# microsoft/Tokenizer

Measured on AMD Instinct MI355X. Metric: input MB/s encoded (cl100k_base), higher is better.
Workload: dtype u8

## Files before the change

tokenizer_amd/csrc/tkz_api.cpp:

```cpp
#include <algorithm>
#include <cstdio>
#include <cstdlib>
#include <cstring>
#include <atomic>
#include <chrono>
#include <memory>
#include <mutex>
#include <thread>
#include <string>
#include <unordered_map>
#include <unordered_set>
#include <vector>

#include "../../include/tkz.h"
#include "tkz_adapt.h"
#include "tkz_bpe.h"
#include "tkz_corpus.h"
#include "tkz_kernels.h"
#include "tkz_pretok.h"
#include "tkz_promo_select.h"
#include "tkz_sdma.h"
#include "tkz_vocab.h"

namespace {
// ... 650 lines not shown
constexpr int64_t kForkMaxLong = int64_t(1) << 20;
constexpr int64_t kForkMaxLongTail = int64_t(1) << 21, kForkTailShare = 2048;
void side_streams(tkz_encoder* e, Workspace* ws, int64_t total, tkz::Launch* L) {
    const bool short_queue = ws->last_lq_total >= 0 && (ws->last_lq_total <= kForkMaxLong || (ws->last_lq_total <= kForkMaxLongTail && ws->last_coop * kForkTailShare >= ws->last_lq_total));
    if (total <= e->latency_bytes || !short_queue) return;
    if (!ws->fork_token) { int none = 0; ws->fork_token = g_fork_in_flight.compare_exchange_strong(none, 1); }
    bool ok = ws->fork_token;
    for (hipStream_t* st : {&ws->st_side, &ws->st_side2}) if (!*st && hipStreamCreateWithFlags(st, hipStreamNonBlocking) != hipSuccess) { *st = nullptr; ok = false; }
    for (hipEvent_t* ev : {&ws->ev_fork, &ws->ev_join, &ws->ev_join2}) if (!*ev && hipEventCreateWithFlags(ev, hipEventDisableTiming) != hipSuccess) { *ev = nullptr; ok = false; }
    if (ok) { L->side = ws->st_side; L->side2 = ws->st_side2; L->ev_fork = ws->ev_fork; L->ev_join = ws->ev_join; L->ev_join2 = ws->ev_join2; }
    else (void)hipGetLastError();
}

int64_t sizing_sample(int64_t ntiles) {
    int64_t min_sub = (int64_t(64) << 20) / tkz::kSub;
    { const char* v = getenv("TKZ_SIZING_MIN_SUB"); if (v && atoll(v) > 0) min_sub = atoll(v); }
    return ntiles >= min_sub ? std::min<int64_t>(ntiles, std::max<int64_t>(ntiles / 16, min_sub / 16)) : -1;
}

tkz_status arm_learning(tkz_encoder* e, Workspace* ws, const BatchCall& c, bool first, TkzTables* T) {
    using namespace tkz;
    const int64_t total = c.total;
    const hipStream_t stream = c.stream;
    {
        std::lock_guard<std::mutex> lock(e->mu);
        bool others = false;
        for (Workspace* w : e->pool) if (w != ws && w->busy) others = true;
        const AdaptPolicy::Arm arm = e->policy.may_learn(total, first && !ws->learning, c.may_learn(), e->T.memo_n != 0, e->T.max_rank < (int32_t)kPromoFlag, e->promo_items.size(), others);
        if (arm != AdaptPolicy::Arm::No && e->t_memo_hits.ensure((size_t)e->memo_slots * 4, &e->bytes_allocated) == hipSuccess &&
            e->t_long_log.ensure((size_t)kLongLogCap * kLongLogDwords * 4 + 64, &e->bytes_allocated) == hipSuccess) {
            const bool clear = arm == AdaptPolicy::Arm::YesClearMemo;
            if (!clear || (hipMemsetAsync(e->t_memo.p, 0, size_t(e->memo_slots) * sizeof(TkzMemoSlot), stream) == hipSuccess && hipStreamSynchronize(stream) == hipSuccess)) {
                ws->learn_window_start = e->policy.window_armed(clear);
                ws->learning = true;
            }
        }
        *T = e->T;
    }
    if (ws->learning) {
        T->memo_hits = e->t_memo_hits.as<uint32_t>();
        T->memo_hits_sparse = total >= (int64_t(64) << 20) ? 1u : 0u;
        if (ws->learn_window_start && first) {
            HIP_TRY(hipMemsetAsync(T->memo_hits, 0, (size_t)e->memo_slots * 4, stream));
            HIP_TRY(hipMemsetAsync(e->t_long_log.as<char>() + (size_t)kLongLogCap * kLongLogDwords * 4, 0, 64, stream));
        }
    }
    return TKZ_OK;
}

tkz::EncodeParams bind_params(Workspace* ws, const uint8_t* d_bytes, const int64_t* d_offs, int64_t n_docs, int64_t total) {
    using namespace tkz;
    char* cb = ws->w_counters.as<char>();
    EncodeParams P{};
    P.bytes = d_bytes; P.total = total; P.startbits = ws->w_startbits.as<uint64_t>(); P.docbits = ws->w_docbits.as<uint64_t>(); P.nwords = total / 64 + 1;
    P.offs = d_offs; P.n_docs = n_docs;
    P.tmp = ws->w_tmp.as<int32_t>(); P.dense = ws->w_dense.as<int32_t>(); P.tile_count = ws->w_tcount.as<int32_t>();
    P.prank = ws->w_prank.as<int32_t>(); P.prank_cap = (int64_t)(ws->w_prank.cap / 4); P.pcount = ws->w_pcount.as<int32_t>(); P.pbase = ws->w_pbase.as<int64_t>();
    P.mlist = ws->w_mlist.as<uint32_t>(); P.mquad = ws->w_mquad.as<uint4>(); P.mcap = ws->mcap; P.mcount = ws->w_mcount.as<uint32_t>();
    P.docord_base = ws->w_dbase.as<int64_t>(); P.doc_tok = ws->w_doctok.as<int32_t>(); P.counters = ws->w_counters.as<int32_t>();
    P.giant_q = ws->w_gq.as<int64_t>(); P.giant_cap = total / kArenaPiece + 1; P.giant_cnt = ws->w_gcnt.as<int32_t>();
    P.giant_count = reinterpret_cast<unsigned long long*>(cb + offsetof(CounterBlock, heavy_count));
    P.giant_ticket = reinterpret_cast<unsigned long long*>(cb + offsetof(CounterBlock, giant_ticket));
    P.heavy_flag = ws->w_heavyq.as<uint8_t>(); P.nsub = (total + kSub - 1) / kSub;
    P.pool = ws->w_pool.as<int32_t>(); P.pool_head = reinterpret_cast<unsigned long long*>(cb + offsetof(CounterBlock, pool_head)); P.pool_cap = (int64_t)(ws->w_pool.cap / 4);
    return P;
}

#ifdef TKZ_DEVPROF
unsigned long long* g_devprof = nullptr;
tkz_status devprof_arm(tkz::EncodeParams* P, hipStream_t stream) {
    { const char* ab = getenv("TKZ_DEV_ABLATE"); P->ablate = ab ? atoi(ab) : 0; }
    if (P->ablate & 16) {
        if (!g_devprof) { HIP_TRY(hipMalloc((void**)&g_devprof, 64 * 8)); }
        HIP_TRY(hipMemsetAsync(g_devprof, 0, 64 * 8, stream));
    }
    P->devprof = g_devprof;
    return TKZ_OK;
}
tkz_status devprof_report() {
    if (!g_devprof || !getenv("TKZ_DEV_ABLATE") || !(atoi(getenv("TKZ_DEV_ABLATE")) & 16)) return TKZ_OK;
    unsigned long long h[64];
    HIP_TRY(hipMemcpy(h, g_devprof, sizeof h, hipMemcpyDeviceToHost));
    const double w = h[0] ? (double)h[0] : 1.0;
    fprintf(stderr, "[tkz devprof] k_probe waves %llu  clock ticks/wave: total %.0f  load+compact %.0f  short batches %.0f  mid batches %.0f | mid pieces/wave %.1f pieces/wave %.1f\n",
            h[0], h[1] / w, h[2] / w, h[3] / w, h[4] / w, h[5] / w, h[6] / w);
    if (h[51]) fprintf(stderr, "[tkz devprof] k_probe lane-cycle table, per sub-tile: load+compact %.0f ticks (64 lanes) | 13+-byte pre-pass %.0f ticks, %.1f pieces in %.2f passes of 64 (lane use %.3f) | main loop: first bucket %.0f ticks at lane use %.3f (%.2f batches of 64, %.1f pieces), second bucket %.0f ticks for %.1f lanes (%.3f of the lanes of the iterations that run it: %.2f of %.2f iterations), records and lists %.0f ticks at lane use %.3f\n",
                       h[2] / w, h[4] / w, h[5] / w, (double)((h[5] + 63 * h[0]) / 64) / w, h[5] ? (double)h[5] / (64.0 * (double)((h[5] + 63 * h[0]) / 64)) : 0.0,
                       h[48] / w, (double)h[52] / (64.0 * (double)h[51]), h[51] / w, h[52] / w, h[49] / w, h[53] / w, h[54] ? (double)h[53] / (128.0 * (double)h[54]) : 0.0, h[54] / w, (double)((h[51] + 1) / 2) / w,
                       h[50] / w, (double)h[52] / (64.0 * (double)h[51]));
    if (h[8]) fprintf(stderr, "[tkz devprof] k_giant_merge pieces %llu  clock ticks/piece: rounds in global memory %.0f  the tail %.0f | bytes/piece %.0f tokens/piece %.0f | slowest piece %llu ticks | global rounds/piece %.2f | parts/piece when the tail took over %.0f\n",
                      h[8], (double)h[9] / h[8], (double)h[10] / h[8], (double)h[11] / h[8], (double)h[12] / h[8], h[13], (double)h[14] / h[8], (double)h[7] / h[8]);
    if (h[8]) fprintf(stderr, "[tkz devprof] slowest giant piece: %llu bytes -> %llu tokens, global rounds %llu (%llu ticks), bytes first/middle/last %02llx %02llx %02llx\n",
                      h[24], h[27], h[25], h[28], h[29] & 255, (h[29] >> 8) & 255, (h[29] >> 16) & 255);
    if (h[32]) fprintf(stderr, "[tkz devprof] k_merge_long waves %llu units %llu  ticks/wave %.0f | of all ticks: sort %.3f batch formation %.3f bytes %.3f first level %.3f merges %.3f emission %.3f | fast batches %llu lanes/batch %.1f steps/batch %.1f merges/lane %.2f lane use in the merge loop %.3f ticks/step %.0f\n",
                       h[32], h[44], (double)h[33] / h[32], (double)h[34] / h[33], (double)h[35] / h[33], (double)h[36] / h[33], (double)h[37] / h[33], (double)h[38] / h[33], (double)h[39] / h[33],
                       h[40], (double)h[41] / (h[40] ? h[40] : 1), (double)h[42] / (h[40] ? h[40] : 1), (double)h[43] / (h[41] ? h[41] : 1), (double)h[43] / (64.0 * (h[42] ? h[42] : 1)), (double)h[38] / (h[42] ? h[42] : 1));
    if (h[16]) fprintf(stderr, "[tkz devprof] tail: batches %llu merges %llu (%.2f a batch) proposals/batch %.1f | rounds for chains of equal pairs %llu | ticks/batch %.0f | longest tail: %llu batches, %llu ticks\n",
                       h[16], h[17], (double)h[17] / h[16], (double)h[18] / h[16], h[19], (double)h[22] / h[16], h[20], h[23]);
    return TKZ_OK;
}
#else
tkz_status devprof_arm(tkz::EncodeParams*, hipStream_t) { return TKZ_OK; }
tkz_status devprof_report() { return TKZ_OK; }
#endif

tkz_status enqueue_attempt(tkz_encoder* e, Workspace* ws, const tkz::Launch& L, const TkzTables& T, const BatchCall& c, bool marks_reused, int64_t nsample,
                           bool* pieces_over) {
    using namespace tkz;
    const hipStream_t stream = L.stream;
    const uint8_t* const d_bytes = c.d_bytes;
    const int64_t* const d_offs = c.d_offs;
    const int64_t n_docs = c.n_docs, total = c.total;
    PiecesOut* const po = c.pieces;
    const int64_t nwords = total / 64 + 1, ntiles = (total + kSub - 1) / kSub;
    int32_t* counters = ws->w_counters.as<int32_t>();
    char* cb = ws->w_counters.as<char>();
    uint64_t* docbits = ws->w_docbits.as<uint64_t>();
    uint64_t* startbits = ws->w_startbits.as<uint64_t>();
    const SpecialCall* const special = c.literals();
    if (marks_reused) {
        HIP_TRY(hipMemsetAsync(ws->w_zero.p, 0, 256, stream));
        if (!c.bitmap_only()) HIP_TRY(hipMemsetAsync(ws->w_heavyq.p, 0, (size_t)(ws->w_zero.as<char>() + ws->zero_bytes - ws->w_heavyq.as<char>()), stream));
    } else {
        if (c.ingest) launch_ingest(L, c.ingest->h_bytes, total, const_cast<uint8_t*>(d_bytes), c.ingest->h_offs, n_docs + 1, const_cast<int64_t*>(d_offs), ws->w_zero.p, (int64_t)ws->zero_bytes);
        else if (ws->zero_bytes <= (size_t(8) << 20)) launch_ingest(L, nullptr, 0, nullptr, nullptr, 0, nullptr, ws->w_zero.p, (int64_t)ws->zero_bytes);
        else HIP_TRY(hipMemsetAsync(ws->w_zero.p, 0, ws->zero_bytes, stream));
        launch_docmark(L, d_offs, n_docs, total, docbits, counters);
        const uint64_t* isobits = docbits;
        const int64_t* iso_offs = d_offs;
        int64_t n_iso = n_docs;
        if (special) {
            for (DevBuf* b : {&ws->w_candbits, &ws->w_segbits, &ws->w_specbits, &ws->w_endbits}) HIP_TRY(b->ensure((size_t)(nwords + 8) * 8, &ws->bytes_allocated));
            launch_lit_scan(L, d_bytes, total, docbits, nwords, e->LIT, special->allowed, ws->w_candbits.as<uint64_t>(), ws->w_segbits.as<uint64_t>(),
                            ws->w_specbits.as<uint64_t>(), ws->w_endbits.as<uint64_t>(), reinterpret_cast<unsigned long long*>(cb + offsetof(CounterBlock, n_literals)), c.d_repl);
            isobits = ws->w_segbits.as<uint64_t>();
            if (e->pretok_seq || e->pattern == TKZ_PATTERN_O200K || e->pattern == TKZ_PATTERN_O200K_DOTNET) {
                int64_t* nseg = reinterpret_cast<int64_t*>(cb + offsetof(CounterBlock, ndocstarts));
                launch_doccount2(L, isobits, isobits, nwords, total, ntiles, ws->w_dcount.as<int32_t>(), ws->w_pcount.as<int32_t>());
                launch_scan2(L, ntiles, ws->w_bsum.as<int64_t>(), ws->w_dcount.as<int32_t>(), ws->w_dbase.as<int64_t>(), nseg, 1, nullptr, nullptr, nullptr, 1, -1);
                HIP_TRY(hipMemcpyAsync(&ws->h_counters->ndocstarts, nseg, 8, hipMemcpyDeviceToHost, stream));
                HIP_TRY(hipStreamSynchronize(stream));
                ws->n_seg = ws->h_counters->ndocstarts;
                HIP_TRY(ws->w_segoffs.ensure((size_t)(ws->n_seg + 2) * 8, &ws->bytes_allocated));
                launch_seg_offsets(L, isobits, nwords, total, ntiles, ws->w_dbase.as<int64_t>(), ws->n_seg, ws->w_segoffs.as<int64_t>());
                iso_offs = ws->w_segoffs.as<int64_t>();
                n_iso = ws->n_seg;
            }
        }
        if (!c.pretokenizes()) {
            HIP_TRY(hipMemcpyAsync(startbits, docbits, (size_t)nwords * 8, hipMemcpyDeviceToDevice, stream));
        } else if (e->pretok_seq) {
            HIP_TRY(hipMemcpyAsync(startbits, isobits, (size_t)nwords * 8, hipMemcpyDeviceToDevice, stream));
            launch_pretok_seq(L, e->pattern, d_bytes, iso_offs, n_iso, total, startbits, T.bmp_class, counters);
        } else {
            HIP_TRY(ws->w_xq.ensure((size_t)(nwords / kRowsPerWave + 4) * 16, &ws->bytes_allocated));
            launch_pretok_rows(L, e->pattern, d_bytes, iso_offs, n_iso, total, isobits, startbits, nwords, T.bmp_class, counters,
                               ws->w_xq.as<int64_t>(), reinterpret_cast<unsigned long long*>(cb + offsetof(CounterBlock, xcount)));
        }
        if (c.pretokenizes() && e->case_equiv && e->pattern == TKZ_PATTERN_CL100K) launch_case_equiv_fix(L, d_bytes, total, isobits, startbits);
        if (special) launch_lit_fix(L, startbits, isobits, ws->w_specbits.as<uint64_t>(), ws->w_endbits.as<uint64_t>(), nwords);
    }
    if (c.bitmap_only()) {
        HIP_TRY(hipMemcpyAsync(c.d_bitmap, startbits, (size_t)nwords * 8, hipMemcpyDeviceToDevice, stream));
    } else {
        EncodeParams P = bind_params(ws, d_bytes, d_offs, n_docs, total);
        P.lane_piece = kLanePiece;
        P.latency = total <= e->latency_bytes ? 1 : 0;
        P.tc_atomic = (L.side || P.latency) ? 1 : 0;
        if (L.side && nsample < 0) ++ws->forked_batches;
        P.coop_cap = total / P.lane_piece + 64;
// ... 1945 lines not shown
```

tokenizer_amd/csrc/tkz_kernels.hip:

```cpp
#include "tkz_kernels.h"

#include <type_traits>

#include "tkz_bpe.h"
#include "tkz_classes.h"
#include "tkz_corpus.h"
#include "tkz_pretok.h"
#include "tkz_simt.h"

namespace tkz {

TKZ_KERNEL(256) void k_docmark(const int64_t* offs, int64_t n_items, int64_t total, uint64_t* bits, int32_t* counters) {
    const int64_t stride = simt::nblocks() * simt::nthreads();
    for (int64_t d = simt::bid() * simt::nthreads() + simt::tid(); d <= n_items; d += stride) {
        const int64_t pos = offs[d];
        bool ok = pos >= 0 && pos <= total;
        if (d == 0) ok = ok && pos == 0;
        if (d == n_items) ok = ok && pos == total;
        else ok = ok && pos <= offs[d + 1];
        if (!ok) { simt::atomic_or((unsigned*)&counters[0], (unsigned)kErrOffsets); continue; }
        const int64_t w = pos >> 6;
        if (d > 0) { const int64_t prev = offs[d - 1]; if (prev >= 0 && prev <= pos && (prev >> 6) == w) continue; }
        uint64_t m = 1ull << (pos & 63);
        int64_t cur = pos;
// ... 352 lines not shown
        if (lane == 0) st = start0;
        int bad = 0;
        if (t0 < b1) {
            int64_t v = t0;
            int64_t d = doc_of(v);
            if (lane == 0) { for (int back = 0; v > offs[d] && v > wlo && back < 3 && (wb(v) & 0xC0) == 0x80; ++back) --v; }
            else { for (int k = 0; k < 3 && v < t1 && v > offs[d] && v < offs[d + 1] && (wb(v) & 0xC0) == 0x80; ++k) ++v; }
            while (v < t1) {
                while (offs[d + 1] <= v) ++d;
                const int64_t a = offs[d], e = offs[d + 1];
                TkzDoc doc; doc.b = win + (a - wlo); doc.n = (e < cut ? e : cut) - a; doc.bmp = bmp; doc.by_code_point = pattern == TKZ_PAT_O200K;
                const TkzChar ch = tkz_doc_char(doc, v - a);
                bad |= ch.bad;
                v += ch.len;
            }
        }
        if (simt::ballot(bad != 0)) { if (lane == 0) simt::atomic_or((unsigned*)&counters[0], (unsigned)kErrUtf8); continue; }
        if (st < lim) {
            int64_t pos = st, d = doc_of(st), curw = -1;
            uint64_t acc = 0;
            while (pos < lim) {
                while (offs[d + 1] <= pos) ++d;
                const int64_t a = offs[d], e = offs[d + 1];
                TkzDoc doc; doc.b = win + (a - wlo); doc.n = (e < cut ? e : cut) - a; doc.bmp = bmp; doc.by_code_point = pattern == TKZ_PAT_O200K;
                if (pos >= b0) {
                    if ((pos >> 6) != curw) {
                        if (acc) simt::atomic_or64((unsigned long long*)&startbits[curw], acc);
                        curw = pos >> 6; acc = 0;
                    }
                    acc |= 1ull << (pos & 63);
                }
                pos = a + tkz_match_at(pattern, doc, pos - a);
            }
            if (acc) simt::atomic_or64((unsigned long long*)&startbits[curw], acc);
        }
    }
}

TKZ_KERNEL(256) void k_pretok_seq(const uint8_t* bytes, const int64_t* offs, int64_t n_docs, int64_t total, uint64_t* startbits,
                                  int pattern, const uint8_t* bmp, int32_t* counters) {
    const int64_t stride = simt::nblocks() * simt::nthreads();
    for (int64_t d = simt::bid() * simt::nthreads() + simt::tid(); d < n_docs; d += stride) {
        const int64_t a = offs[d], b = offs[d + 1];
        if (b <= a || a < 0 || b > total) continue;
        TkzDoc doc; doc.b = bytes + a; doc.n = b - a; doc.bmp = bmp; doc.by_code_point = pattern == TKZ_PAT_O200K;
        int bad = 0;
        for (int64_t p = 0; p < doc.n;) { const TkzChar c = tkz_doc_char(doc, p); bad |= c.bad; p += c.len; }
        if (bad) { simt::atomic_or((unsigned*)&counters[0], (unsigned)kErrUtf8); continue; }
        int64_t curw = -1; uint64_t acc = 0;
        for (int64_t p = 0; p < doc.n;) {
            const int64_t g = a + p;
            if ((g >> 6) != curw) {
                if (acc) simt::atomic_or64((unsigned long long*)&startbits[curw], acc);
                curw = g >> 6; acc = 0;
            }
            acc |= 1ull << (g & 63);
            p = tkz_match_at(pattern, doc, p);
        }
        if (acc) simt::atomic_or64((unsigned long long*)&startbits[curw], acc);
    }
}

constexpr uint32_t kPrMiss = 1u << 31, kPrMark = 1u << 30, kPrLong = 1u << 29, kPrGiant = 1u << 28;
constexpr uint32_t kPrRankMask = (1u << 28) - 1u;
constexpr uint32_t kMrDone = 1u << 31, kMrDense = 1u << 30, kMrInline = 1u << 29;
constexpr int kMrLenShift = 10, kMrCntShift = 12;
constexpr uint32_t kMrOffMask = (1u << kMrCntShift) - 1u;
static_assert(kDenseCap <= (1 << kMrCntShift) && kSub <= (1 << kMrLenShift), "the offset field of a result entry");
#ifndef TKZ_PROBE_U
#define TKZ_PROBE_U 2
#endif
#ifndef TKZ_MS_THREADS
#define TKZ_MS_THREADS 256
#endif
#ifndef TKZ_PROBE_OCC
#define TKZ_PROBE_OCC 8
#endif
constexpr int kGroup = kMergeGroup;
constexpr int kMsThreads = TKZ_MS_THREADS;
#ifndef TKZ_PROBE_PER
#define TKZ_PROBE_PER 1
#endif
constexpr int kProbePer = TKZ_PROBE_PER;
constexpr int kMidMax = kSub / (TKZ_SHORT_KEY_MAX + 1) + 2;

TKZ_DEV int64_t tkz_xcd_block(int64_t b, int64_t nblocks) { return (b & 7) * (nblocks >> 3) + (b >> 3); }

template <int BITS>
TKZ_DEV int tkz_wave_scan(int v, int* total) {
    const uint64_t below = tkz_lowmask(simt::lane());
    int pre = 0, tot = 0;
#pragma unroll
    for (int j = 0; j < BITS; ++j) {
        const uint64_t m = simt::ballot((v >> j) & 1);
        pre += tkz_popc64(m & below) << j;
        tot += tkz_popc64(m) << j;
    }
    *total = tot;
    return pre;
}

TKZ_DEV int tkz_wave_scan_sum(int v, int* total) {
    const int x = simt::scan_inclusive(v);
    *total = simt::last_lane(x);
    return x - v;
}

TKZ_DEV uint32_t tkz_key_dword(const uint32_t* s_bytes, int s, int len, int i) {
    const int w = (s >> 2) + i;
    const uint32_t x = simt::alignbit(s_bytes[w + 1], s_bytes[w], (uint32_t)(s & 3) * 8u);
    const int nb = len - 4 * i;
    return nb >= 4 ? x : (nb <= 0 ? 0u : (x & ((1u << (8 * nb)) - 1u)));
}

constexpr int kProbeLdsBytes = (kSub + kHalo) + 2 * (kSub + 2) + 2 * kMidMax + 4 * kMidMax + 4 * (kSub / 32);
constexpr int kProbeLdsQuads = (kProbeLdsBytes + 15) / 16;
struct ProbeLds { uint32_t* bytes; uint16_t* pstart; uint16_t* mid; uint32_t* midres; uint32_t* mark; const uint4* kmask; uint32_t* spec ; };
TKZ_DEV ProbeLds tkz_probe_lds(uint4* wave_quads, const uint4* kmask) {
    ProbeLds L;
    uint8_t* b = reinterpret_cast<uint8_t*>(wave_quads);
    L.bytes = reinterpret_cast<uint32_t*>(b); b += kSub + kHalo;
    L.midres = reinterpret_cast<uint32_t*>(b); b += 4 * kMidMax;
    L.mark = reinterpret_cast<uint32_t*>(b); b += 4 * (kSub / 32);
    L.pstart = reinterpret_cast<uint16_t*>(b); b += 2 * (kSub + 2);
    L.mid = reinterpret_cast<uint16_t*>(b);
    L.kmask = kmask;
    L.spec = nullptr;
    return L;
}
TKZ_DEV void tkz_probe_kmask_init(uint4* s_kmask) {
    if (simt::tid() <= TKZ_SHORT_KEY_MAX) {
        const int len = simt::tid();
        uint32_t m[3];
        for (int i = 0; i < 3; ++i) { const int nb = len - 4 * i; m[i] = nb >= 4 ? 0xFFFFFFFFu : (nb <= 0 ? 0u : ((1u << (8 * nb)) - 1u)); }
        uint4 v; v.x = m[0]; v.y = m[1]; v.z = m[2]; v.w = 0;
        s_kmask[len] = v;
    }
}
struct ProbeText { uint4 v0, v1; };
static_assert((kSub + kHalo) / 16 <= 128, "two 16-byte loads per lane cover the sub-tile and its halo");
TKZ_DEV void tkz_probe_request_text(const EncodeParams& P, int64_t sub, ProbeText* tx) {
    const int lane = simt::lane();
    const int64_t base = sub * kSub;
    uint4 v0, v1;
    v0.x = v0.y = v0.z = v0.w = 0; v1 = v0;
    const int64_t p0 = base + 16 * (int64_t)lane, p1 = base + 16 * (int64_t)(lane + 64);
    if (p0 + 16 <= P.total) v0 = tkz_load16_nt(P.bytes + p0);
    else {
        uint32_t w[4] = {0, 0, 0, 0};
        for (int j = 0; j < 16; ++j) if (p0 + j < P.total) w[j >> 2] |= (uint32_t)P.bytes[p0 + j] << (8 * (j & 3));
        v0.x = w[0]; v0.y = w[1]; v0.z = w[2]; v0.w = w[3];
    }
    if (lane + 64 < (kSub + kHalo) / 16) {
        if (p1 + 16 <= P.total) v1 = tkz_load16_nt(P.bytes + p1);
        else {
            uint32_t w[4] = {0, 0, 0, 0};
            for (int j = 0; j < 16; ++j) if (p1 + j < P.total) w[j >> 2] |= (uint32_t)P.bytes[p1 + j] << (8 * (j & 3));
            v1.x = w[0]; v1.y = w[1]; v1.z = w[2]; v1.w = w[3];
        }
    }
    tx->v0 = v0; tx->v1 = v1;
}
TKZ_DEV bool tkz_bits_any(const uint64_t* rw, int64_t nrw, int64_t bit, int len) {
    const int64_t wa = bit >> 6, wb = (bit + len - 1) >> 6;
    for (int64_t w = wa; w <= wb && w < nrw; ++w) {
        uint64_t m = rw[w];
        if (w == wa) m &= ~tkz_lowmask((int)(bit & 63));
        if (w == wb) m &= tkz_lowmask((int)((bit + len - 1) & 63) + 1);
        if (m) return true;
    }
    return false;
}
TKZ_DEV bool tkz_lit_replaced(const uint32_t* meta, int i, const uint64_t* rw, int64_t nrw, int64_t bit, int len) {
    return rw && ((meta[kLitFffdHead + (i >> 5)] >> (i & 31)) & 1u) && tkz_bits_any(rw, nrw, bit, len);
}
TKZ_DEV int32_t tkz_lit_id(const EncodeParams& P, const uint8_t* sb, const uint8_t* gb, int s, int len, int64_t abs) {
    const uint8_t* tx = s + len <= kSub + kHalo ? sb + s : gb + s;
    for (int i = 0; i < P.n_lit; ++i) {
        const uint32_t m = P.lit_meta[kLitMetaHead + 2 * i];
        if ((int)(m >> 16) != len) continue;
        const uint8_t* lit = P.lit_blob + (m & 0xFFFFu);
        int k = 0;
        while (k < len && lit[k] == tx[k]) ++k;
        if (k == len && !tkz_lit_replaced(P.lit_meta, i, P.lit_repl, P.nwords, abs, len)) return (int32_t)P.lit_meta[kLitMetaHead + 2 * i + 1];
    }
    return TKZ_RANK_NONE;
}
template <bool REPORT, bool SPECIAL = false>
TKZ_DEV void tkz_probe_subtile(const TkzTables& T, const EncodeParams& P, int64_t sub, const ProbeLds& LD, ProbeText& tx, int64_t next) {
    const int lane = simt::lane();
    uint32_t* s_bytes = LD.bytes;
    uint16_t* s_pstart = LD.pstart;
    uint16_t* s_mid = LD.mid;
    uint32_t* s_midres = LD.midres;
    uint32_t* s_mark = LD.mark;
    const uint4* s_kmask = LD.kmask;
    const uint8_t* sb = reinterpret_cast<const uint8_t*>(s_bytes);
    const int64_t base = sub * kSub;
    const int nb = (int)(P.total - base < kSub ? P.total - base : kSub);
    const uint8_t* gbase = P.bytes + base;
    const bool prof = TKZ_DEV_FLAG(P, 16);
    long long t_0 = prof ? simt::clock() : 0, t_1 = 0, t_2 = 0, t_3 = 0;
    uint4 v0 = tx.v0, v1 = tx.v1;
    uint64_t myword = 0, mymark = 0;
    uint64_t myspec = 0;
    if (lane < kSub / 64) {
        const int64_t w = sub * (kSub / 64) + lane;
        if (w < P.nwords) { myword = P.startbits[w]; mymark = P.docbits[w]; if (SPECIAL) myspec = P.specbits[w]; }
    }
    const int64_t from = base + nb, w0 = from >> 6;
    uint64_t ahead = (w0 + lane < P.nwords) ? P.startbits[w0 + lane] : 0ull;
    const int64_t pb = P.pbase[sub];
    { uint4* s4 = reinterpret_cast<uint4*>(s_bytes); s4[lane] = v0; if (lane + 64 < (kSub + kHalo) / 16) s4[lane + 64] = v1; }
    if (next >= 0) tkz_probe_request_text(P, next, &tx);
    if (lane < kSub / 64) {
        const int lim = nb - lane * 64;
        if (lim <= 0) myword = 0; else if (lim < 64) myword &= tkz_lowmask(lim);
        s_mark[2 * lane] = (uint32_t)mymark; s_mark[2 * lane + 1] = (uint32_t)(mymark >> 32);
        if (SPECIAL) { LD.spec[2 * lane] = (uint32_t)myspec; LD.spec[2 * lane + 1] = (uint32_t)(myspec >> 32); }
    }
    int64_t last_end;
    {
        int64_t found = -1;
        for (int64_t c = 0; found < 0; ++c) {
            const int64_t w = w0 + c * 64 + lane;
            uint64_t v = c == 0 ? ahead : (w < P.nwords ? P.startbits[w] : 0);
            if (w == w0) v &= ~tkz_lowmask((int)(from & 63));
            const uint64_t any = simt::ballot(v != 0);
            if (any) {
                const int src = tkz_ctz64(any);
                const uint32_t lo = simt::shflu((uint32_t)v, src), hi = simt::shflu((uint32_t)(v >> 32), src);
                found = ((w0 + c * 64 + src) << 6) + tkz_ctz64(((uint64_t)hi << 32) | lo);
            } else if (w0 + (c + 1) * 64 >= P.nwords) found = P.total;
        }
        last_end = found;
    }
    const int last_end_rel = (int)(last_end - base < 2 * kSub + 2 ? last_end - base : 2 * kSub + 2);
    const uint32_t wlo = simt::shflu((uint32_t)myword, lane >> 2), whi = simt::shflu((uint32_t)(myword >> 32), lane >> 2);
    const uint32_t bits16 = (uint32_t)(((((uint64_t)whi << 32) | wlo) >> (16 * (lane & 3))) & 0xFFFFull);
    int np;
    {
        int off = tkz_wave_scan<5>(tkz_popc32(bits16), &np);
        for (uint32_t b = bits16; b; b &= b - 1) s_pstart[off++] = (uint16_t)(16 * lane + tkz_ctz32(b));
        if (lane == 0) s_pstart[np] = (uint16_t)last_end_rel;
    }
    (void)simt::ballot(true);
    if (prof) t_1 = simt::clock();
    const char* tb0 = reinterpret_cast<const char*>(T.short_slots);
    const uint32_t mid_off = (uint32_t)(reinterpret_cast<const char*>(T.mid_slots) - tb0);
    int nmid = 0;
#pragma unroll 1
    for (int k0 = 0; k0 < np; k0 += 64) {
        const int k = k0 + lane;
        int len = 0;
        if (k < np) len = (int)s_pstart[k + 1] - (int)s_pstart[k];
        const uint64_t midm = simt::ballot(len > TKZ_SHORT_KEY_MAX && len <= kArenaPiece);
        if ((midm >> lane) & 1ull) s_mid[nmid + tkz_popc64(midm & tkz_lowmask(lane))] = (uint16_t)k;
        nmid += tkz_popc64(midm);
    }
    (void)simt::ballot(true);
#pragma unroll 1
    for (int m0 = 0; m0 < nmid; m0 += 64) {
        const bool valid = m0 + lane < nmid;
        int s = 0, len = 13;
        uint32_t kk[7] = {0, 0, 0, 0, 0, 0, 0}, oa = 0, ob = 0;
        if (valid) {
            const int k = s_mid[m0 + lane];
            s = s_pstart[k];
            len = (int)s_pstart[k + 1] - s;
        }
        const bool is_lit = SPECIAL && valid && ((LD.spec[s >> 5] >> (s & 31)) & 1u);
        const bool is_mid = valid && len <= TKZ_MID_KEY_MAX && !is_lit;
        if (is_mid) {
#pragma unroll
            for (int i = 0; i < 7; ++i) kk[i] = tkz_key_dword(s_bytes, s, len, i);
            uint32_t s1, s2;
            tkz_mid_slots(T, kk, (uint32_t)len, &s1, &s2);
            oa = mid_off + 32u * s1; ob = mid_off + 32u * s2;
        }
        const uint4 a0 = tkz_load16(tb0 + oa), a1 = tkz_load16(tb0 + oa + 16u), b0 = tkz_load16(tb0 + ob), b1 = tkz_load16(tb0 + ob + 16u);
        int32_t rank = TKZ_RANK_NONE;
        if (is_mid) rank = tkz_match_mid(kk, (uint32_t)len, a0, a1, b0, b1);
        else if (is_lit) rank = tkz_lit_id(P, sb, gbase, s, len, base + s);
        else if (valid) {
            if (s + len <= kSub + kHalo) rank = tkz_lookup_long(T, [&](int i) -> uint32_t { return sb[s + i]; }, (uint32_t)len);
            else rank = tkz_lookup_long(T, [&](int i) -> uint32_t { return gbase[s + i]; }, (uint32_t)len);
        }
        if (valid) s_midres[m0 + lane] = (uint32_t)rank;
    }
    (void)simt::ballot(true);
    if (prof) t_2 = simt::clock();
    uint32_t* const ml = P.mlist + sub * (int64_t)P.mcap;
    uint4* const mq = P.mquad + sub * (int64_t)P.mcap;
    int ns = 0, nl = 0, midseen = 0;
    int promo_extra = 0;
    bool giant = false, coopl = false;
    constexpr int U = TKZ_PROBE_U;
#ifdef TKZ_DEVPROF
    long long pf_first = 0, pf_second = 0, pf_emit = 0, pf_t = 0;
    int pf_batches = 0, pf_valid = 0, pf_want2 = 0, pf_iters2 = 0;
#define TKZ_PROBE_MARK(acc) do { if (prof) { const long long pf_now = simt::clock(); acc += pf_now - pf_t; pf_t = pf_now; } } while (0)
    if (prof) pf_t = simt::clock();
#else
#define TKZ_PROBE_MARK(acc) do { } while (0)
#endif
#pragma unroll 1
    for (int k0 = 0; k0 < np; k0 += 64 * U) {
        int ps[U], plen[U];
        uint32_t hs[U], kw0[U], kw1[U], kw2[U];
        uint4 a0[U], a1[U];
#pragma unroll
        for (int u = 0; u < U; ++u) {
            const int k = k0 + 64 * u + lane;
            ps[u] = 0; plen[u] = 0;
            if (k < np) { ps[u] = s_pstart[k]; plen[u] = (int)s_pstart[k + 1] - ps[u]; }
            const int s = ps[u], w = s >> 2;
            const uint32_t sh = (uint32_t)(s & 3) * 8u;
            const uint32_t d0 = s_bytes[w], d1 = s_bytes[w + 1], d2 = s_bytes[w + 2], d3 = s_bytes[w + 3];
            const bool is_short = plen[u] >= 1 && plen[u] <= TKZ_SHORT_KEY_MAX;
            const uint4 km = s_kmask[is_short ? plen[u] : 0];
            kw0[u] = simt::alignbit(d1, d0, sh) & km.x; kw1[u] = simt::alignbit(d2, d1, sh) & km.y; kw2[u] = simt::alignbit(d3, d2, sh) & km.z;
            const uint32_t slot = tkz_short_slot_first(T, kw0[u], kw1[u], kw2[u], (uint32_t)plen[u], &hs[u]);
            const uint32_t oa = is_short ? 16u * slot : 0u;
            a0[u] = tkz_load16(tb0 + oa); a1[u] = tkz_load16(tb0 + oa + 16u);
        }
        int32_t rk[U];
        bool more = false;
#pragma unroll
        for (int u = 0; u < U; ++u) {
            const bool is_short = plen[u] >= 1 && plen[u] <= TKZ_SHORT_KEY_MAX;
            rk[u] = tkz_match_short2x(kw0[u], kw1[u], kw2[u], (uint32_t)plen[u], a0[u], a1[u]);
            if (SPECIAL && is_short && ((LD.spec[ps[u] >> 5] >> (ps[u] & 31)) & 1u)) rk[u] = tkz_lit_id(P, sb, gbase, ps[u], plen[u], base + ps[u]);
            more = more || (is_short && rk[u] == TKZ_RANK_NONE);
        }
        bool two_pass = simt::ballot(more) != 0;
        TKZ_PROBE_MARK(pf_first);
#ifdef TKZ_DEVPROF
        if (prof) {
            for (int u = 0; u < U; ++u) { const int nv = np - (k0 + 64 * u); if (nv > 0) { ++pf_batches; pf_valid += nv < 64 ? nv : 64; } }
            for (int u = 0; u < U; ++u) pf_want2 += tkz_popc64(simt::ballot(plen[u] >= 1 && plen[u] <= TKZ_SHORT_KEY_MAX && rk[u] == TKZ_RANK_NONE));
            pf_iters2 += two_pass ? 1 : 0;
            pf_t = simt::clock();
        }
#endif
        if (two_pass) {
#pragma unroll
            for (int u = 0; u < U; ++u) {
                const bool want = plen[u] >= 1 && plen[u] <= TKZ_SHORT_KEY_MAX && rk[u] == TKZ_RANK_NONE;
                if (want) {
                    const uint32_t ob = 16u * tkz_short_slot_second(T, hs[u]);
                    a0[u] = tkz_load16(tb0 + ob); a1[u] = tkz_load16(tb0 + ob + 16u);
                }
            }
#pragma unroll
            for (int u = 0; u < U; ++u) {
                const bool want = plen[u] >= 1 && plen[u] <= TKZ_SHORT_KEY_MAX && rk[u] == TKZ_RANK_NONE;
                if (want) rk[u] = tkz_match_short2x(kw0[u], kw1[u], kw2[u], (uint32_t)plen[u], a0[u], a1[u]);
            }
        }
        TKZ_PROBE_MARK(pf_second);
#pragma unroll
        for (int u = 0; u < U; ++u) {
            const int k = k0 + 64 * u + lane;
            const bool valid = k < np;
            const int s = ps[u], len = plen[u];
            const bool is_mid = len > TKZ_SHORT_KEY_MAX && len <= kArenaPiece;
            const uint64_t midm = simt::ballot(is_mid);
            int32_t rank = rk[u];
            if (is_mid) rank = (int32_t)s_midres[midseen + tkz_popc64(midm & tkz_lowmask(lane))];
            midseen += tkz_popc64(midm);
            const bool is_giant = len > kArenaPiece;
            const bool miss = valid && !is_giant && rank == TKZ_RANK_NONE;
            if (P.pextra) {
                const uint32_t ex = (valid && !is_giant && !miss && ((uint32_t)rank & kPromoFlag)) ? (((uint32_t)rank >> kPromoCntShift) & 3u) : 0u;
                promo_extra += (int)ex;
            }
            const bool miss_s = miss && len <= kShortMax, miss_l = miss && len > kShortMax;
            const uint64_t sm = simt::ballot(miss_s), lm = simt::ballot(miss_l);
            const int is_ = ns + tkz_popc64(sm & tkz_lowmask(lane)), il = nl + tkz_popc64(lm & tkz_lowmask(lane));
            ns += tkz_popc64(sm); nl += tkz_popc64(lm);
            const uint32_t ent = (uint32_t)s | ((uint32_t)(len - 1) << kMrLenShift);
            if (miss_s && is_ + nl < P.mcap) {
                ml[is_] = ent;
                uint4 kq; kq.x = kw0[u]; kq.y = kw1[u]; kq.z = kw2[u]; kq.w = 0;
                if (len > TKZ_SHORT_KEY_MAX) { kq.x = tkz_key_dword(s_bytes, s, len, 0); kq.y = tkz_key_dword(s_bytes, s, len, 1); kq.z = tkz_key_dword(s_bytes, s, len, 2); kq.w = tkz_key_dword(s_bytes, s, len, 3); }
                mq[is_] = kq;
            }
            if (miss_l && il + ns < P.mcap) ml[P.mcap - 1 - il] = ent;
            uint32_t rec = ((s_mark[s >> 5] >> (s & 31)) & 1u) ? kPrMark : 0u;
            if (REPORT) giant = giant || (miss_l && len > kSmallLanePiece);
            else coopl = coopl || (miss_l && len > P.lane_piece);
            if (is_giant) { rec |= kPrMiss | kPrGiant | (uint32_t)s; giant = giant || valid; }
            else if (miss) rec |= kPrMiss | (miss_l ? (kPrLong | (uint32_t)il) : (uint32_t)is_);
            else rec |= (uint32_t)rank;
            if (valid && pb + k < P.prank_cap) tkz_store_nt(&P.prank[pb + k], (int32_t)rec);
        }
        TKZ_PROBE_MARK(pf_emit);
    }
#undef TKZ_PROBE_MARK
#ifdef TKZ_DEVPROF
    if (prof && lane == 0) {
        simt::atomic_add64(&P.devprof[48], (unsigned long long)pf_first); simt::atomic_add64(&P.devprof[49], (unsigned long long)pf_second);
        simt::atomic_add64(&P.devprof[50], (unsigned long long)pf_emit); simt::atomic_add64(&P.devprof[51], (unsigned long long)pf_batches);
        simt::atomic_add64(&P.devprof[52], (unsigned long long)pf_valid); simt::atomic_add64(&P.devprof[53], (unsigned long long)pf_want2);
        simt::atomic_add64(&P.devprof[54], (unsigned long long)pf_iters2);
    }
#endif
    if (prof && lane == 0) {
        t_3 = simt::clock();
        simt::atomic_add64(&P.devprof[0], 1); simt::atomic_add64(&P.devprof[1], (unsigned long long)(t_3 - t_0));
        simt::atomic_add64(&P.devprof[2], (unsigned long long)(t_1 - t_0)); simt::atomic_add64(&P.devprof[3], (unsigned long long)(t_3 - t_2));
        simt::atomic_add64(&P.devprof[4], (unsigned long long)(t_2 - t_1)); simt::atomic_add64(&P.devprof[5], (unsigned long long)nmid);
        simt::atomic_add64(&P.devprof[6], (unsigned long long)np);
    }
    const uint32_t f = (nl ? 1u : 0u) | (simt::ballot(giant) ? 2u : 0u) | (simt::ballot(coopl) ? 4u : 0u);
    if (P.pextra) { int tot; (void)tkz_wave_scan_sum(promo_extra, &tot); promo_extra = tot; }
    if (lane == 0) {
        P.heavy_flag[sub] = (uint8_t)f;
        P.mcount[sub] = (uint32_t)ns | ((uint32_t)nl << 16);
        if (P.pextra) P.pextra[sub] = promo_extra;
        if (!REPORT && P.tc_atomic) P.tile_count[sub] = 0;
        if (REPORT && ns + nl > P.mcap) { simt::atomic_or((unsigned*)&P.counters[0], (unsigned)kErrMissCap); simt::atomic_max((unsigned*)&P.counters[1], (unsigned)(ns + nl)); }
        if (pb + np > P.prank_cap) simt::atomic_or((unsigned*)&P.counters[0], (unsigned)kErrCapacity);
    }
}
TKZ_KERNEL_OCC(256, TKZ_PROBE_OCC) void k_probe(TkzTables T, EncodeParams P) {
    TKZ_SHARED uint4 s_wave[kThreads / 64][kProbeLdsQuads];
    TKZ_SHARED uint4 s_kmask[TKZ_SHORT_KEY_MAX + 1];
    tkz_probe_kmask_init(s_kmask);
    simt::sync();
    const int64_t sub0 = (tkz_xcd_block(simt::bid(), simt::nblocks()) * (kThreads / 64) + simt::wave()) * kProbePer;
    if (sub0 >= P.nsub) return;
    const ProbeLds LD = tkz_probe_lds(s_wave[simt::wave()], s_kmask);
    ProbeText tx;
    tkz_probe_request_text(P, sub0, &tx);
#pragma unroll 1
    for (int it = 0; it < kProbePer && sub0 + it < P.nsub; ++it) {
        const int64_t nxt = (it + 1 < kProbePer && sub0 + it + 1 < P.nsub) ? sub0 + it + 1 : -1;
        tkz_probe_subtile<false>(T, P, sub0 + it, LD, tx, nxt);
        (void)simt::ballot(true);
    }
}

TKZ_KERNEL_OCC(256, TKZ_PROBE_OCC) void k_probe_special(TkzTables T, EncodeParams P) {
    TKZ_SHARED uint4 s_wave[kThreads / 64][kProbeLdsQuads];
    TKZ_SHARED uint4 s_kmask[TKZ_SHORT_KEY_MAX + 1];
    TKZ_SHARED uint32_t s_spec[kThreads / 64][kSub / 32];
    tkz_probe_kmask_init(s_kmask);
    simt::sync();
    const int64_t sub0 = (tkz_xcd_block(simt::bid(), simt::nblocks()) * (kThreads / 64) + simt::wave()) * kProbePer;
    if (sub0 >= P.nsub) return;
    ProbeLds LD = tkz_probe_lds(s_wave[simt::wave()], s_kmask);
    LD.spec = s_spec[simt::wave()];
    ProbeText tx;
    tkz_probe_request_text(P, sub0, &tx);
#pragma unroll 1
    for (int it = 0; it < kProbePer && sub0 + it < P.nsub; ++it) {
        const int64_t nxt = (it + 1 < kProbePer && sub0 + it + 1 < P.nsub) ? sub0 + it + 1 : -1;
        tkz_probe_subtile<false, true>(T, P, sub0 + it, LD, tx, nxt);
        (void)simt::ballot(true);
    }
}

struct alignas(4) TkzDwords4 { uint32_t x, y, z, w; };
TKZ_DEV void tkz_load_piece16(const uint8_t* bytes, int64_t total, int64_t abs, uint32_t* pw) {
    const int64_t a0 = abs & ~(int64_t)3;
    const uint32_t sh = (uint32_t)(abs & 3) * 8u;
    uint32_t w[5];
    if (a0 + 20 <= total) {
        const TkzDwords4 v = *reinterpret_cast<const TkzDwords4*>(bytes + a0);
        w[0] = v.x; w[1] = v.y; w[2] = v.z; w[3] = v.w;
        w[4] = *reinterpret_cast<const uint32_t*>(bytes + a0 + 16);
    } else {
#pragma unroll
        for (int i = 0; i < 5; ++i) {
            const int64_t p = a0 + 4 * i;
            if (p + 4 <= total) w[i] = *reinterpret_cast<const uint32_t*>(bytes + p);
            else { w[i] = 0; for (int j = 0; j < 4; ++j) if (p + j < total) w[i] |= (uint32_t)bytes[p + j] << (8 * j); }
        }
    }
#pragma unroll
    for (int i = 0; i < 4; ++i) pw[i] = simt::alignbit(w[i + 1], w[i], sh);
}

TKZ_HD uint32_t tkz_result_entry(bool dense, int cnt, int off) { return kMrDone | (dense ? kMrDense : 0u) | ((uint32_t)(cnt - 1) << kMrCntShift) | (uint32_t)off; }
TKZ_HD uint32_t tkz_result_inline(int cnt) { return kMrDone | kMrInline | ((uint32_t)(cnt - 1) << kMrCntShift); }
TKZ_HD int tkz_result_cnt(uint32_t r) { return (int)((r >> kMrCntShift) & 1023u) + 1; }
TKZ_HD int tkz_result_off(uint32_t r) { return (int)(r & kMrOffMask); }

template <int N, class Pre>
TKZ_DEV int tkz_find_list(const Pre* pre, int g) {
    int q = 0;
#pragma unroll
    for (int step = N / 2; step >= 1; step >>= 1) if (pre[q + step] <= g) q += step;
    return q;
// ... 2769 lines not shown
```

Baseline: 269,700.

## Defer probe misses to compacted exception passes and stage records in LDS

```diff
diff --git a/tokenizer_amd/csrc/tkz_api.cpp b/tokenizer_amd/csrc/tkz_api.cpp
--- a/tokenizer_amd/csrc/tkz_api.cpp
+++ b/tokenizer_amd/csrc/tkz_api.cpp
@@ -756,10 +756,10 @@
     unsigned long long h[64];
     HIP_TRY(hipMemcpy(h, g_devprof, sizeof h, hipMemcpyDeviceToHost));
     const double w = h[0] ? (double)h[0] : 1.0;
-    fprintf(stderr, "[tkz devprof] k_probe waves %llu  clock ticks/wave: total %.0f  load+compact %.0f  short batches %.0f  mid batches %.0f | mid pieces/wave %.1f pieces/wave %.1f\n",
-            h[0], h[1] / w, h[2] / w, h[3] / w, h[4] / w, h[5] / w, h[6] / w);
-    if (h[51]) fprintf(stderr, "[tkz devprof] k_probe lane-cycle table, per sub-tile: load+compact %.0f ticks (64 lanes) | 13+-byte pre-pass %.0f ticks, %.1f pieces in %.2f passes of 64 (lane use %.3f) | main loop: first bucket %.0f ticks at lane use %.3f (%.2f batches of 64, %.1f pieces), second bucket %.0f ticks for %.1f lanes (%.3f of the lanes of the iterations that run it: %.2f of %.2f iterations), records and lists %.0f ticks at lane use %.3f\n",
-                       h[2] / w, h[4] / w, h[5] / w, (double)((h[5] + 63 * h[0]) / 64) / w, h[5] ? (double)h[5] / (64.0 * (double)((h[5] + 63 * h[0]) / 64)) : 0.0,
+    fprintf(stderr, "[tkz devprof] k_probe waves %llu  clock ticks/wave: total %.0f  load+compact %.0f  short batches and record stores %.0f  exception passes %.0f | exceptions/wave %.1f in %.2f passes, pieces/wave %.1f\n",
+            h[0], h[1] / w, h[2] / w, h[3] / w, h[4] / w, h[5] / w, h[55] / w, h[6] / w);
+    if (h[51]) fprintf(stderr, "[tkz devprof] k_probe lane-cycle table, per sub-tile: load+compact %.0f ticks (64 lanes) | exception passes %.0f ticks, %.1f exceptions in %.2f passes of 64 (lane use %.3f) | main loop: first bucket %.0f ticks at lane use %.3f (%.2f batches of 64, %.1f pieces), second bucket %.0f ticks for %.1f lanes (%.3f of the lanes of the iterations that run it: %.2f of %.2f iterations), records into the stage %.0f ticks at lane use %.3f\n",
+                       h[2] / w, h[4] / w, h[5] / w, h[55] / w, h[55] ? (double)h[5] / (64.0 * (double)h[55]) : 0.0,
                        h[48] / w, (double)h[52] / (64.0 * (double)h[51]), h[51] / w, h[52] / w, h[49] / w, h[53] / w, h[54] ? (double)h[53] / (128.0 * (double)h[54]) : 0.0, h[54] / w, (double)((h[51] + 1) / 2) / w,
                        h[50] / w, (double)h[52] / (64.0 * (double)h[51]));
     if (h[8]) fprintf(stderr, "[tkz devprof] k_giant_merge pieces %llu  clock ticks/piece: rounds in global memory %.0f  the tail %.0f | bytes/piece %.0f tokens/piece %.0f | slowest piece %llu ticks | global rounds/piece %.2f | parts/piece when the tail took over %.0f\n",
diff --git a/tokenizer_amd/csrc/tkz_kernels.hip b/tokenizer_amd/csrc/tkz_kernels.hip
--- a/tokenizer_amd/csrc/tkz_kernels.hip
+++ b/tokenizer_amd/csrc/tkz_kernels.hip
@@ -458,7 +458,6 @@
 #define TKZ_PROBE_PER 1
 #endif
 constexpr int kProbePer = TKZ_PROBE_PER;
-constexpr int kMidMax = kSub / (TKZ_SHORT_KEY_MAX + 1) + 2;
 
 TKZ_DEV int64_t tkz_xcd_block(int64_t b, int64_t nblocks) { return (b & 7) * (nblocks >> 3) + (b >> 3); }
 
@@ -489,17 +488,21 @@
     return nb >= 4 ? x : (nb <= 0 ? 0u : (x & ((1u << (8 * nb)) - 1u)));
 }
 
-constexpr int kProbeLdsBytes = (kSub + kHalo) + 2 * (kSub + 2) + 2 * kMidMax + 4 * kMidMax + 4 * (kSub / 32);
+constexpr int kProbeChunk = 256;
+static_assert(kProbeChunk == 4 * 64 && kProbeChunk % (64 * TKZ_PROBE_U) == 0 && kRecordLine % 4 == 0 && (kSub + kHalo) % 16 == 0,
+              "a chunk is whole iterations of the main loop and one quad a lane; a sub-tile's records start on a 64-byte line; the stage is 16-byte aligned");
+constexpr int kProbeLdsBytes = (kSub + kHalo) + 2 * (kSub + 2) + 4 * kProbeChunk + 2 * kProbeChunk + 4 * (kSub / 32);
 constexpr int kProbeLdsQuads = (kProbeLdsBytes + 15) / 16;
-struct ProbeLds { uint32_t* bytes; uint16_t* pstart; uint16_t* mid; uint32_t* midres; uint32_t* mark; const uint4* kmask; uint32_t* spec ; };
+static_assert(4 * kProbeLdsQuads * 16 + 16 * (TKZ_SHORT_KEY_MAX + 1) + 4 * 4 * (kSub / 32) <= 160 * 1024 / 8, "k_probe / k_probe_special: 8 workgroups of 4 wavefronts a CU");
+struct ProbeLds { uint32_t* bytes; uint16_t* pstart; uint16_t* exc; uint32_t* stage; uint32_t* mark; const uint4* kmask; uint32_t* spec ; };
 TKZ_DEV ProbeLds tkz_probe_lds(uint4* wave_quads, const uint4* kmask) {
     ProbeLds L;
     uint8_t* b = reinterpret_cast<uint8_t*>(wave_quads);
     L.bytes = reinterpret_cast<uint32_t*>(b); b += kSub + kHalo;
-    L.midres = reinterpret_cast<uint32_t*>(b); b += 4 * kMidMax;
+    L.stage = reinterpret_cast<uint32_t*>(b); b += 4 * kProbeChunk;
     L.mark = reinterpret_cast<uint32_t*>(b); b += 4 * (kSub / 32);
-    L.pstart = reinterpret_cast<uint16_t*>(b); b += 2 * (kSub + 2);
-    L.mid = reinterpret_cast<uint16_t*>(b);
+    L.exc = reinterpret_cast<uint16_t*>(b); b += 2 * kProbeChunk;
+    L.pstart = reinterpret_cast<uint16_t*>(b);
     L.kmask = kmask;
     L.spec = nullptr;
     return L;
@@ -562,13 +565,22 @@
     }
     return TKZ_RANK_NONE;
 }
+TKZ_DEV int32_t tkz_match_short2v(uint32_t k0, uint32_t k1, uint32_t k2, uint32_t len, uint4 a0, uint4 a1) {
+    uint32_t d0 = (a0.x ^ k0) | (a0.y ^ k1) | (a0.z ^ k2) | ((a0.w >> TKZ_SHORT_RANK_BITS) ^ len);
+    uint32_t d1 = (a1.x ^ k0) | (a1.y ^ k1) | (a1.z ^ k2) | ((a1.w >> TKZ_SHORT_RANK_BITS) ^ len);
+#ifndef TKZ_HOSTEMU
+    asm volatile("" : "+v"(d0), "+v"(d1));
+#endif
+    const uint32_t r = d0 == 0 ? a0.w : a1.w;
+    return ((d0 == 0 || d1 == 0) && len != 0) ? (int32_t)(r & TKZ_SHORT_RANK_MASK) : TKZ_RANK_NONE;
+}
 template <bool REPORT, bool SPECIAL = false>
 TKZ_DEV void tkz_probe_subtile(const TkzTables& T, const EncodeParams& P, int64_t sub, const ProbeLds& LD, ProbeText& tx, int64_t next) {
     const int lane = simt::lane();
     uint32_t* s_bytes = LD.bytes;
     uint16_t* s_pstart = LD.pstart;
-    uint16_t* s_mid = LD.mid;
-    uint32_t* s_midres = LD.midres;
+    uint16_t* s_exc = LD.exc;
+    uint32_t* s_stage = LD.stage;
     uint32_t* s_mark = LD.mark;
     const uint4* s_kmask = LD.kmask;
     const uint8_t* sb = reinterpret_cast<const uint8_t*>(s_bytes);
@@ -576,7 +588,8 @@
     const int nb = (int)(P.total - base < kSub ? P.total - base : kSub);
     const uint8_t* gbase = P.bytes + base;
     const bool prof = TKZ_DEV_FLAG(P, 16);
-    long long t_0 = prof ? simt::clock() : 0, t_1 = 0, t_2 = 0, t_3 = 0;
+    long long t_0 = prof ? simt::clock() : 0, t_1 = 0, t_3 = 0, t_exc = 0;
+    int nexc_all = 0, nexc_passes = 0;
     uint4 v0 = tx.v0, v1 = tx.v1;
     uint64_t myword = 0, mymark = 0;
     uint64_t myspec = 0;
@@ -624,51 +637,9 @@
     if (prof) t_1 = simt::clock();
     const char* tb0 = reinterpret_cast<const char*>(T.short_slots);
     const uint32_t mid_off = (uint32_t)(reinterpret_cast<const char*>(T.mid_slots) - tb0);
-    int nmid = 0;
-#pragma unroll 1
-    for (int k0 = 0; k0 < np; k0 += 64) {
-        const int k = k0 + lane;
-        int len = 0;
-        if (k < np) len = (int)s_pstart[k + 1] - (int)s_pstart[k];
-        const uint64_t midm = simt::ballot(len > TKZ_SHORT_KEY_MAX && len <= kArenaPiece);
-        if ((midm >> lane) & 1ull) s_mid[nmid + tkz_popc64(midm & tkz_lowmask(lane))] = (uint16_t)k;
-        nmid += tkz_popc64(midm);
-    }
-    (void)simt::ballot(true);
-#pragma unroll 1
-    for (int m0 = 0; m0 < nmid; m0 += 64) {
-        const bool valid = m0 + lane < nmid;
-        int s = 0, len = 13;
-        uint32_t kk[7] = {0, 0, 0, 0, 0, 0, 0}, oa = 0, ob = 0;
-        if (valid) {
-            const int k = s_mid[m0 + lane];
-            s = s_pstart[k];
-            len = (int)s_pstart[k + 1] - s;
-        }
-        const bool is_lit = SPECIAL && valid && ((LD.spec[s >> 5] >> (s & 31)) & 1u);
-        const bool is_mid = valid && len <= TKZ_MID_KEY_MAX && !is_lit;
-        if (is_mid) {
-#pragma unroll
-            for (int i = 0; i < 7; ++i) kk[i] = tkz_key_dword(s_bytes, s, len, i);
-            uint32_t s1, s2;
-            tkz_mid_slots(T, kk, (uint32_t)len, &s1, &s2);
-            oa = mid_off + 32u * s1; ob = mid_off + 32u * s2;
-        }
-        const uint4 a0 = tkz_load16(tb0 + oa), a1 = tkz_load16(tb0 + oa + 16u), b0 = tkz_load16(tb0 + ob), b1 = tkz_load16(tb0 + ob + 16u);
-        int32_t rank = TKZ_RANK_NONE;
-        if (is_mid) rank = tkz_match_mid(kk, (uint32_t)len, a0, a1, b0, b1);
-        else if (is_lit) rank = tkz_lit_id(P, sb, gbase, s, len, base + s);
-        else if (valid) {
-            if (s + len <= kSub + kHalo) rank = tkz_lookup_long(T, [&](int i) -> uint32_t { return sb[s + i]; }, (uint32_t)len);
-            else rank = tkz_lookup_long(T, [&](int i) -> uint32_t { return gbase[s + i]; }, (uint32_t)len);
-        }
-        if (valid) s_midres[m0 + lane] = (uint32_t)rank;
-    }
-    (void)simt::ballot(true);
-    if (prof) t_2 = simt::clock();
     uint32_t* const ml = P.mlist + sub * (int64_t)P.mcap;
     uint4* const mq = P.mquad + sub * (int64_t)P.mcap;
-    int ns = 0, nl = 0, midseen = 0;
+    int ns = 0, nl = 0, nexc = 0;
     int promo_extra = 0;
     bool giant = false, coopl = false;
     constexpr int U = TKZ_PROBE_U;
@@ -706,7 +677,6 @@
         for (int u = 0; u < U; ++u) {
             const bool is_short = plen[u] >= 1 && plen[u] <= TKZ_SHORT_KEY_MAX;
             rk[u] = tkz_match_short2x(kw0[u], kw1[u], kw2[u], (uint32_t)plen[u], a0[u], a1[u]);
-            if (SPECIAL && is_short && ((LD.spec[ps[u] >> 5] >> (ps[u] & 31)) & 1u)) rk[u] = tkz_lit_id(P, sb, gbase, ps[u], plen[u], base + ps[u]);
             more = more || (is_short && rk[u] == TKZ_RANK_NONE);
         }
         bool two_pass = simt::ballot(more) != 0;
@@ -731,20 +701,67 @@
 #pragma unroll
             for (int u = 0; u < U; ++u) {
                 const bool want = plen[u] >= 1 && plen[u] <= TKZ_SHORT_KEY_MAX && rk[u] == TKZ_RANK_NONE;
-                if (want) rk[u] = tkz_match_short2x(kw0[u], kw1[u], kw2[u], (uint32_t)plen[u], a0[u], a1[u]);
+                if (want) rk[u] = tkz_match_short2v(kw0[u], kw1[u], kw2[u], (uint32_t)plen[u], a0[u], a1[u]);
             }
         }
         TKZ_PROBE_MARK(pf_second);
 #pragma unroll
         for (int u = 0; u < U; ++u) {
             const int k = k0 + 64 * u + lane;
-            const bool valid = k < np;
-            const int s = ps[u], len = plen[u];
-            const bool is_mid = len > TKZ_SHORT_KEY_MAX && len <= kArenaPiece;
-            const uint64_t midm = simt::ballot(is_mid);
-            int32_t rank = rk[u];
-            if (is_mid) rank = (int32_t)s_midres[midseen + tkz_popc64(midm & tkz_lowmask(lane))];
-            midseen += tkz_popc64(midm);
+            const int s = ps[u];
+            const int32_t rank = rk[u];
+            bool hit = rank != TKZ_RANK_NONE;
+            if (SPECIAL) hit = hit && !((LD.spec[s >> 5] >> (s & 31)) & 1u);
+            const bool exc = k < np && !hit;
+            if (P.pextra) {
+                const uint32_t ex = (hit && ((uint32_t)rank & kPromoFlag)) ? (((uint32_t)rank >> kPromoCntShift) & 3u) : 0u;
+                promo_extra += (int)ex;
+            }
+            const int kc = (k0 & (kProbeChunk - 1)) + 64 * u + lane;
+            s_stage[kc] = (uint32_t)rank | (((s_mark[s >> 5] >> (s & 31)) & 1u) << 30);
+            const uint64_t em = simt::ballot(exc);
+            if (exc) s_exc[nexc + tkz_popc64(em & tkz_lowmask(lane))] = (uint16_t)kc;
+            nexc += tkz_popc64(em);
+        }
+        TKZ_PROBE_MARK(pf_emit);
+        if (((k0 + 64 * U) & (kProbeChunk - 1)) != 0 && k0 + 64 * U < np) continue;
+        const int c0 = k0 & ~(kProbeChunk - 1);
+        (void)simt::ballot(true);
+        const long long t_e0 = prof ? simt::clock() : 0;
+#pragma unroll 1
+        for (int e0 = 0; e0 < nexc; e0 += 64) {
+            const bool valid = e0 + lane < nexc;
+            int kc = 0, s = 0, len = 0;
+            if (valid) {
+                kc = s_exc[e0 + lane];
+                s = s_pstart[c0 + kc];
+                len = (int)s_pstart[c0 + kc + 1] - s;
+            }
+            const bool is_lit = SPECIAL && valid && ((LD.spec[s >> 5] >> (s & 31)) & 1u);
+            const bool is_mid = len > TKZ_SHORT_KEY_MAX && len <= TKZ_MID_KEY_MAX && !is_lit;
+            int32_t rank = TKZ_RANK_NONE;
+            uint32_t kk[7] = {0, 0, 0, 0, 0, 0, 0};
+            if (valid && len <= TKZ_MID_KEY_MAX) {
+#pragma unroll
+                for (int i = 0; i < 4; ++i) kk[i] = tkz_key_dword(s_bytes, s, len, i);
+            }
+            if (simt::ballot(is_mid)) {
+                uint32_t oa = 0, ob = 0;
+                if (is_mid) {
+#pragma unroll
+                    for (int i = 4; i < 7; ++i) kk[i] = tkz_key_dword(s_bytes, s, len, i);
+                    uint32_t s1, s2;
+                    tkz_mid_slots(T, kk, (uint32_t)len, &s1, &s2);
+                    oa = mid_off + 32u * s1; ob = mid_off + 32u * s2;
+                }
+                const uint4 a0 = tkz_load16(tb0 + oa), a1 = tkz_load16(tb0 + oa + 16u), b0 = tkz_load16(tb0 + ob), b1 = tkz_load16(tb0 + ob + 16u);
+                if (is_mid) rank = tkz_match_mid(kk, (uint32_t)len, a0, a1, b0, b1);
+            }
+            if (is_lit) rank = tkz_lit_id(P, sb, gbase, s, len, base + s);
+            else if (len > TKZ_MID_KEY_MAX && len <= kArenaPiece) {
+                if (s + len <= kSub + kHalo) rank = tkz_lookup_long(T, [&](int i) -> uint32_t { return sb[s + i]; }, (uint32_t)len);
+                else rank = tkz_lookup_long(T, [&](int i) -> uint32_t { return gbase[s + i]; }, (uint32_t)len);
+            }
             const bool is_giant = len > kArenaPiece;
             const bool miss = valid && !is_giant && rank == TKZ_RANK_NONE;
             if (P.pextra) {
@@ -758,20 +775,38 @@
             const uint32_t ent = (uint32_t)s | ((uint32_t)(len - 1) << kMrLenShift);
             if (miss_s && is_ + nl < P.mcap) {
                 ml[is_] = ent;
-                uint4 kq; kq.x = kw0[u]; kq.y = kw1[u]; kq.z = kw2[u]; kq.w = 0;
-                if (len > TKZ_SHORT_KEY_MAX) { kq.x = tkz_key_dword(s_bytes, s, len, 0); kq.y = tkz_key_dword(s_bytes, s, len, 1); kq.z = tkz_key_dword(s_bytes, s, len, 2); kq.w = tkz_key_dword(s_bytes, s, len, 3); }
+                uint4 kq; kq.x = kk[0]; kq.y = kk[1]; kq.z = kk[2]; kq.w = kk[3];
                 mq[is_] = kq;
             }
             if (miss_l && il + ns < P.mcap) ml[P.mcap - 1 - il] = ent;
             uint32_t rec = ((s_mark[s >> 5] >> (s & 31)) & 1u) ? kPrMark : 0u;
             if (REPORT) giant = giant || (miss_l && len > kSmallLanePiece);
             else coopl = coopl || (miss_l && len > P.lane_piece);
-            if (is_giant) { rec |= kPrMiss | kPrGiant | (uint32_t)s; giant = giant || valid; }
+            if (is_giant) { rec |= kPrMiss | kPrGiant | (uint32_t)s; giant = true; }
             else if (miss) rec |= kPrMiss | (miss_l ? (kPrLong | (uint32_t)il) : (uint32_t)is_);
             else rec |= (uint32_t)rank;
-            if (valid && pb + k < P.prank_cap) tkz_store_nt(&P.prank[pb + k], (int32_t)rec);
-        }
-        TKZ_PROBE_MARK(pf_emit);
+            if (valid) s_stage[kc] = rec;
+        }
+        if (prof) { t_exc += simt::clock() - t_e0; nexc_all += nexc; nexc_passes += (nexc + 63) >> 6; }
+        nexc = 0;
+        (void)simt::ballot(true);
+        {
+            const int n = np - c0 < kProbeChunk ? np - c0 : kProbeChunk, r0 = 4 * lane;
+            if (r0 < n) {
+                const uint4 v = reinterpret_cast<const uint4*>(s_stage)[lane];
+                const int64_t g = pb + c0 + r0;
+                if (r0 + 4 <= n && g + 4 <= P.prank_cap) tkz_store16_nt(&P.prank[g], v);
+                else {
+                    const uint32_t r[4] = {v.x, v.y, v.z, v.w};
+#pragma unroll
+                    for (int j = 0; j < 4; ++j) if (r0 + j < n && g + j < P.prank_cap) tkz_store_nt(&P.prank[g + j], (int32_t)r[j]);
+                }
+            }
+        }
+        (void)simt::ballot(true);
+#ifdef TKZ_DEVPROF
+        if (prof) pf_t = simt::clock();
+#endif
     }
 #undef TKZ_PROBE_MARK
 #ifdef TKZ_DEVPROF
@@ -785,8 +820,9 @@
     if (prof && lane == 0) {
         t_3 = simt::clock();
         simt::atomic_add64(&P.devprof[0], 1); simt::atomic_add64(&P.devprof[1], (unsigned long long)(t_3 - t_0));
-        simt::atomic_add64(&P.devprof[2], (unsigned long long)(t_1 - t_0)); simt::atomic_add64(&P.devprof[3], (unsigned long long)(t_3 - t_2));
-        simt::atomic_add64(&P.devprof[4], (unsigned long long)(t_2 - t_1)); simt::atomic_add64(&P.devprof[5], (unsigned long long)nmid);
+        simt::atomic_add64(&P.devprof[2], (unsigned long long)(t_1 - t_0)); simt::atomic_add64(&P.devprof[3], (unsigned long long)(t_3 - t_1 - t_exc));
+        simt::atomic_add64(&P.devprof[4], (unsigned long long)t_exc); simt::atomic_add64(&P.devprof[5], (unsigned long long)nexc_all);
+        simt::atomic_add64(&P.devprof[55], (unsigned long long)nexc_passes);
         simt::atomic_add64(&P.devprof[6], (unsigned long long)np);
     }
     const uint32_t f = (nl ? 1u : 0u) | (simt::ballot(giant) ? 2u : 0u) | (simt::ballot(coopl) ? 4u : 0u);
```

After: 272,600 (median of 6 runs). +1.1%, better.
